# raadyn/aztotmd

Hardware: AMD Instinct MI355X
Metric: ns_per_day (higher is better)
Workload: dtype f64; 1 GPU; 1 000 188 Ar, LJ rc 8.5 A, FCC 63^3 a=5.735 jitter 0.15, dt 1 fs, NVE, init_vel zero (BASELINE config '1 000 000 Ar LJ', SURVEY C4); n_atoms=1000188, n_cells=68921, decomposition=single GPU, transport=single GPU, rccl_ranks=0, pair_variant=0, sort_interval=105, sort_violations=0, pair_lists=1, cells_without_list=0, kernel_timing=off

## Files before the change

aztotmd_amd/api.py:

```python
import ctypes as C
import enum
import os
import subprocess

import numpy as np

_HERE = os.path.dirname(os.path.abspath(__file__))
_LIB = None

STAT_FIELDS = ("step", "time", "engTot", "engKin", "engVdW", "engCoul", "engElecField", "engTemp", "engPot", "temperature",
               "posMom", "negMom", "posCross", "negCross", "pressure", "pairs_dropped", "n_cells", "nose_chit", "nose_conint",
               "engBond", "engAngle", "engCoulRec", "engCoulConst", "sort_interval", "sort_violations", "pair_lists", "cells_without_list", "rebuilds", "skin")


class AztotError(RuntimeError):
    def __init__(self, code, msg):
        super().__init__("aztot error %d: %s" % (code, msg))
        self.code = code


class _Species(C.Structure):
    _fields_ = [("name", C.c_char * 8), ("mass_amu", C.c_double), ("charge", C.c_double), ("frozen", C.c_int32),
                ("radA", C.c_double), ("radB", C.c_double), ("mxEng", C.c_double)]

# ... 92 lines not shown
           "aztot_adf_setup", "aztot_adf_sample", "aztot_adf_reset", "aztot_adf_shape", "aztot_adf_edges", "aztot_adf_counts", "aztot_adf_values",
           "aztot_adf_neighbours",
           "aztot_sk_setup", "aztot_sk_sample", "aztot_sk_reset", "aztot_sk_shape", "aztot_sk_vectors", "aztot_sk_amplitudes", "aztot_sk_sums", "aztot_sk_values",
           "aztot_boo_setup", "aztot_boo_sample", "aztot_boo_reset", "aztot_boo_shape", "aztot_boo_per_atom", "aztot_boo_qlm", "aztot_boo_counts", "aztot_boo_values",
           "aztot_last_error", "aztot_version")

RDF_KINDS = {"species": 0, "nuclei": 1}
CN_KINDS = {"species": 0, "nuclei": 1}


class DebugBit(enum.IntFlag):
    DBG_BUILD_PHASE_MASK = 3
    DBG_ALWAYS_CLEANUP = 4
    DBG_FOLD_DRIFT = 8
    DBG_NO_FOLD_DRIFT = 16
    DBG_KICK_EVERY_STEP = 128
    DBG_LARGE_KICK_PATH = 256
    DBG_GENERIC_PAIR = 512
    DBG_KEEP_VDW_CUT_TEST = 1024
    DBG_STAGE_ONLY = 2048
    DBG_SLAB_GRAPH = 4096
    DBG_FIXED_INTERVAL = 8192
    DBG_OVERLAP_HALO = 16384
    DBG_NO_LISTS = 32768
    DBG_SHORT_LISTS = 65536
    DBG_NO_FUSE_NEXT = 131072
    DBG_FUSE_NEXT = 262144
    DBG_CHECK_EVERY_ATOM = 524288
    DBG_LIST_STATS = 2097152
    DBG_KICK_POST_SPLIT = 4194304
# ... 670 lines not shown
```

aztotmd_amd/csrc/device_md.h:

```cpp
#pragma once
#include <cstdint>

namespace aztot {

constexpr int kSpecCap = 16;

struct AtomArrays
{
    double *x, *y, *z;
    double *vx, *vy, *vz;
    double *fx, *fy, *fz;
    double *U, *rad;
    int32_t *type;
    int32_t *id;
};

struct RefPos { double *x, *y, *z; };

struct SpecTable
{
    double mass[kSpecCap], charge[kSpecCap], rMhdt[kSpecCap];
    double radA[kSpecCap], radB[kSpecCap], mxEng[kSpecCap];
    int32_t charged[kSpecCap], frozen[kSpecCap];
};
// ... 48 lines not shown

struct SplitArgs
{
    int n = 1;
    double *fx = nullptr, *fy = nullptr, *fz = nullptr;
    int32_t* arrived = nullptr;
    int capacity = 0;
};

enum DebugBit : unsigned
{
    DBG_BUILD_PHASE_MASK = 3,
    DBG_ALWAYS_CLEANUP = 4,
    DBG_FOLD_DRIFT = 8,
    DBG_NO_FOLD_DRIFT = 16,
    DBG_KICK_EVERY_STEP = 128,
    DBG_LARGE_KICK_PATH = 256,
    DBG_GENERIC_PAIR = 512,
    DBG_KEEP_VDW_CUT_TEST = 1024,
    DBG_STAGE_ONLY = 2048,
    DBG_SLAB_GRAPH = 4096,
    DBG_FIXED_INTERVAL = 8192,
    DBG_OVERLAP_HALO = 16384,
    DBG_NO_LISTS = 32768,
    DBG_SHORT_LISTS = 65536,
    DBG_NO_FUSE_NEXT = 131072,
    DBG_FUSE_NEXT = 262144,
    DBG_CHECK_EVERY_ATOM = 524288,
    DBG_LIST_STATS = 2097152,
    DBG_KICK_POST_SPLIT = 4194304,
// ... 107 lines not shown
```

aztotmd_amd/csrc/engine.h:

```cpp
#pragma once
#include <hip/hip_runtime.h>

#include <algorithm>
#include <memory>
#include <stdexcept>
#include <string>
#include <vector>

#include "device_md.h"
#include "device_resources.h"
#include "list_store.h"
#include "model.h"
#include "msg_layout.h"
#include "samplers.h"

namespace aztot {

struct Counts;
struct PairLists; struct PairLaunch;

struct ArgError : std::runtime_error
{
    using std::runtime_error::runtime_error;
};
// ... 151 lines not shown

    double lastMom_[6] = {0, 0, 0, 0, 0, 0};
    double pressure_ = 0.0;
    long long lastPresStep_ = 0;

    std::unique_ptr<Samplers> samplers_;

    struct BufState { int cur; double* xyz[2][3]; double* alt[2][3]; };
    struct LaunchNotes
    {
        int pairBlocksUsed = 0;
        int blocksEver = 0;
        bool ekinFromPair = false;
        bool lastStepEquil = false;
    } notes_;
    struct GraphSlot { BufState before, after; LaunchNotes notes; hipGraph_t graph = nullptr; hipGraphExec_t exec = nullptr; };
    void adopt_launch_notes(const LaunchNotes& n) { const int ever = std::max(notes_.blocksEver, n.blocksEver); notes_ = n; notes_.blocksEver = ever; }
    std::vector<GraphSlot> graphs_;
    int graphCycle_ = 0;
    bool capturing_ = false;
    void drop_graphs();
    BufState buf_state() const;
    GraphSlot* graph_for_state(int cycle);
    int graph_cycle() const;
    bool can_graph() const;
    void set_buf_state(const BufState& b);

    bool lazyKick_ = false;
    bool kickOwed_ = false;
    bool fuseEpilogue_ = false;
    bool fuseNow_ = false;
// ... 40 lines not shown
```

aztotmd_amd/csrc/engine.hip:

```cpp
#include "engine.h"

#include <algorithm>
#include <cmath>
#include <array>
#include <cstring>
#include <cstddef>
#include <cstdio>
#include <cstdlib>
#include <stdexcept>
#include <tuple>

#include "exchange.h"
#include "bonded.hip.h"
#include "ewald.hip.h"
#include "kernels.hip.h"
#include "pair_tile.hip.h"
#include "pair_list.hip.h"
#include "rdf.hip.h"
#include "cn.hip.h"
#include "adf.hip.h"
#include "sk.hip.h"
#include "tcf.hip.h"
#include "slab.hip.h"

// ... 480 lines not shown
    PairLists probe;
    probe.candCap = probe.candLds = probe.stageLds = candCapNew; probe.iterCap = probe.iterLds = iterCapNew; probe.recBytes = pair_list_rec_bytes(P); probe.waves = waves;
    while (candCapNew > kListMinCand && (pair_list_lds_bytes(P, probe) > ldsMax_ || build_lists_lds_bytes(probe) > ldsMax_))
    {
        candCapNew -= 64;
        probe.candCap = probe.candLds = probe.stageLds = candCapNew;
    }
    while (iterCapNew > 2 * kListMinIter && build_lists_lds_bytes(probe) > ldsMax_) { iterCapNew -= 8; probe.iterCap = probe.iterLds = iterCapNew; }
    const size_t nc = (size_t)P.nCellLocal;
    cand = mem_.alloc<uint32_t>(nc * candCapNew, true, stream_);
    meta = mem_.alloc<int32_t>(4 * nc, false, stream_);
    pairs = mem_.alloc<uint16_t>(nc * (size_t)waves * (size_t)iterCapNew * kWave, true, stream_);
    report = mem_.alloc<int32_t>(LR_COUNT, true, stream_); rel = mem_.alloc<float4>((size_t)capacity_ + kWave, true, stream_);
    candCap = candCapNew; iterCap = iterCapNew;
    candLds = stageLds = candCapNew; iterLds = iterCapNew;
    {
        std::vector<int32_t> mx(4 * nc, 0);
        const int ncy = P.nc[1], ncz = P.nc[2];
        for (size_t c = 0; c < nc; c++)
        {
            const int cz = (int)(c % ncz), cy = (int)((c / ncz) % ncy), lx = (int)(c / ((size_t)ncy * ncz));
            mx[4 * c] = -1; mx[4 * c + 1] = lx | (cy << 10) | (cz << 20);
        }
        HIP_CHECK(hipMemcpyAsync(meta, mx.data(), sizeof(int32_t) * 4 * nc, hipMemcpyHostToDevice, stream_));
        HIP_CHECK(hipStreamSynchronize(stream_));
    }
    on = true;
    if (std::getenv("AZTOT_VERBOSE"))
        std::fprintf(stderr, "aztot: pair lists for %zu cells: %d candidates, %d iterations per cell (%.1f MB), LDS %zu B (list kernel) / %zu B (builder)\n", nc, candCap, iterCap,
                     (double)(nc * ((size_t)candCap * 4 + (size_t)iterCap * 128)) / 1e6, pair_list_lds_bytes(P, pair_lists()), build_lists_lds_bytes(pair_lists()));
// ... 12 lines not shown

void ListStore::release() noexcept
{
    if (stream_) (void)hipStreamSynchronize(stream_);
    mem_.release();
    cand = nullptr; meta = nullptr; pairs = nullptr; report = nullptr; rel = nullptr;
    on = false;
}

PairLists ListStore::pair_lists() const
{
    PairLists pl;
    if (on)
    {
        pl.cand = cand; pl.meta = meta; pl.pairs = pairs; pl.noList = report;
        pl.candCap = candCap; pl.iterCap = iterCap; pl.candLds = candLds; pl.stageLds = stageLds; pl.iterLds = iterLds; pl.recBytes = pair_list_rec_bytes(*P_); pl.entryScale = pair_list_entry_scale(*P_); pl.waves = waves;
        pl.rel = rel;
    }
    return pl;
}

int ListStore::tile_records_for(int maxT) const
{
    constexpr size_t kLdsBlock = 1280;
    PairLists L = pair_lists();
    const bool roomy = P_->nranks == 1 && capacity_ <= 2 * kFuseKickMaxAtoms;
    const int need = std::max(4 * kWave, std::min(candCap, roomy ? maxT + maxT / 16 + 4 : maxT + maxT / 100 + 1));
    if (need <= 4 * kWave) return need;
    L.candLds = need;
    const size_t blocks = (pair_list_lds_bytes(*P_, L) + kLdsBlock - 1) / kLdsBlock;
    int best = need;
    for (int c = need + 1; c <= candCap; c++)
    {
        L.candLds = c;
        if ((pair_list_lds_bytes(*P_, L) + kLdsBlock - 1) / kLdsBlock > blocks) break;
        best = c;
    }
    return best;
}

int ListStore::stage_records_for(int maxStaged) const
{
    return std::max(4 * kWave, std::min(candCap, (maxStaged + maxStaged / 16 + 4 + 127) & ~127));
}

void ListStore::lds_for(const int32_t* rep, int& candLdsNew, int& stageLdsNew, int& iterLdsNew) const
{
    candLdsNew = tile_records_for(rep[LR_MAX_TILE]);
    stageLdsNew = stage_records_for(rep[LR_MAX_STAGED]);
    iterLdsNew = std::max(2 * kListMinIter, std::min(iterCap, (rep[LR_MAX_ITERS] + rep[LR_MAX_ITERS] / 8 + 2 + 7) & ~7));
}

bool ListStore::tighten(const int32_t* rep)
{
    if (rep[LR_TILE_FULL] != 0 || rep[LR_LIST_FULL] != 0 || rep[LR_KEPT_FULL] != 0 || rep[LR_MAX_STAGED] <= 0) return false;
    int c, s, i;
    lds_for(rep, c, s, i);
    if (c >= candLds && s >= stageLds && i >= iterLds) return false;
    candLds = std::min(candLds, c); stageLds = std::min(stageLds, s); iterLds = std::min(iterLds, i);
    return true;
}

ListStore::Verdict ListStore::adapt(const int32_t* rep, unsigned debug)
{
    Verdict v;
    const bool frozen = debug & DBG_SHORT_LISTS;
    if (debug & DBG_LIST_STATS)
    {
        std::fprintf(stderr, "aztot: per cell: %.2f list iterations, %.1f candidates staged, %.1f kept, %.2f atoms\n", (double)rep[LR_SUM_ITERS] / rep[LR_RECORDED],
                     (double)rep[LR_SUM_STAGED] / rep[LR_RECORDED], (double)rep[LR_SUM_CANDS] / rep[LR_RECORDED], (double)rep[LR_SUM_ATOMS] / rep[LR_RECORDED]);
        HIP_CHECK(hipMemset(&report[LR_SUM_ITERS], 0, sizeof(int32_t) * 4));
    }
    HIP_CHECK(hipMemsetAsync(&report[LR_UNLISTED], 0, sizeof(int32_t) * 2, stream_));
    HIP_CHECK(hipMemsetAsync(&report[LR_TILE_FULL], 0, sizeof(int32_t) * 3, stream_));
    const int tileFull = rep[LR_TILE_FULL], keptFull = rep[LR_KEPT_FULL], listFull = rep[LR_LIST_FULL], recorded = rep[LR_RECORDED], unlisted = rep[LR_UNLISTED];
    if (std::getenv("AZTOT_VERBOSE"))
        std::fprintf(stderr, "aztot: lists recorded since the last look: %d cells, %d of them without a list (%d: staging full, %d: tile full, %d: list full); most staged %d of %d (LDS %d), largest tile %d (LDS %d), longest list %d of %d (LDS %d)\n",
                     recorded, unlisted, tileFull, keptFull, listFull, rep[LR_MAX_STAGED], candCap, stageLds, rep[LR_MAX_TILE], candLds, rep[LR_MAX_ITERS], iterCap, iterLds);
    int candLdsNew, stageLdsNew, iterLdsNew;
    lds_for(rep, candLdsNew, stageLdsNew, iterLdsNew);
    if (tileFull > 0) stageLdsNew = std::min(candCap, std::max(stageLdsNew, stageLds + 128));
    if (keptFull > 0) candLdsNew = std::min(candCap, std::max(candLdsNew, candLds + 32));
    if (listFull > 0) iterLdsNew = std::min(iterCap, std::max(iterLdsNew, iterLds + 8));
    if (frozen) { candLdsNew = candLds; stageLdsNew = stageLds; iterLdsNew = iterLds; }
    const int wWant = std::max(waves, waves_wanted((double)rep[LR_MAX_TILE], rep[LR_MAX_ITERS]));
    if (wWant > waves && !forcedWaves_ && !frozen)
    {
        const int itersNew = std::max(2 * kListMinIter, ((int)(rep[LR_MAX_ITERS] * (double)waves / wWant * 1.3) + 8 + 7) & ~7);
        const int candNew = std::max(candCap, kListMinCand * wWant);
        waves = wWant;
        regrow(candNew, itersNew);
        v.rebuild = v.launchChanged = true;
        return v;
    }
    const bool capFull = (tileFull > 0 && stageLds == candCap) || (keptFull > 0 && candLds == candCap) || (listFull > 0 && iterLds == iterCap);
    if (capFull && !frozen && (double)(tileFull + keptFull + listFull) > ((P_->nranks == 1 && growths < 3) ? 0.0 : 0.0005 * (double)recorded))
    {
        const int candNew = tileFull + keptFull > 0 ? std::min(kListCandMax, (candCap * 3 / 2 + 63) & ~63) : candCap;
        const int itersNew = listFull > 0 ? std::min(kListIterMax, (iterCap * 2 + 7) & ~7) : iterCap;
        v.launchChanged = true;
// ... 203 lines not shown
    return variant;
}

PairLaunch Engine::pair_launch(const StepParams& Q) { return PairLaunch{Q, S_, dPots_, cur(), dCounts_, dCellStart_, dPartials_, maxBlocks_, stream_}; }

void Engine::launch_pair()
{
    const int variant = pair_variant();
    int splitBlocks = 0;
    if (variant == 2)
    {
        StepParams Q = P_;
        Q.fuseKick = fuseNow_ ? KICK_SECOND : KICK_NONE;
        const PairLaunch C = pair_launch(Q);
        const bool wantEnergies = stepsLeftInRun_ == 0 || (debug_ & DBG_ENERGIES_EVERY_STEP);
        const PairLists pl = lists_.pair_lists();
        if (overlapHalo_)
        {
            const int plane = P_.nc[1] * P_.nc[2], hw = P_.hw[0];
            PairRange in, lo, hi;
            in.first = 2 * hw * plane; in.n = (P_.ncxLocal - 4 * hw) * plane;
            lo.first = hw * plane; lo.n = hw * plane;
            hi.first = (P_.ncxLocal - 2 * hw) * plane; hi.n = hw * plane;
            const bool lists = candMode_ == 2 && pl.cand;
            int nb = 0;
            auto run = [&](PairRange& r) {
                r.blockBase = nb;
                if (lists)
                {
                    nb += launch_pair_list(C, r, pl, NextStep(), wantEnergies);
// ... 37 lines not shown
                if (fuseNext_) { nx.xn = altXyz_[cur_][0]; nx.yn = altXyz_[cur_][1]; nx.zn = altXyz_[cur_][2]; }
                if (fuseNext_ && fuseNextTstat_) { nx.photons = dPhotons_; nx.uvx = dUvx_; nx.uvy = dUvy_; nx.uvz = dUvz_; pairClosedStep_ = true; }
                else nx.pendingAfter = lazyKick_ ? 1 : -1;
                const bool fold = foldKick_ && skipCleanup && !fuseNext_ && !wantEnergies;
                foldKick_ = false;
                StepParams QL = Q;
                const bool foldDrift = fold && foldDriftOk_;
                if (fold) { QL.fuseKick = foldDrift ? KICK_DRIFT : KICK_BOTH; nx.pendingAfter = 0; kickFolded_ = !foldDrift; }
                if (foldDrift)
                {
                    nx.xd = altXyz_[cur_][0]; nx.yd = altXyz_[cur_][1]; nx.zd = altXyz_[cur_][2];
                    nx.driftBlocks = div_up(div_up(capacity_, 2), kBlock);
                    if (profile_ && !capturing_) timers_.count("fold_drift");
                }
                const PairLaunch CL = pair_launch(QL);
                timed("pair_list", [&] { splitBlocks = launch_pair_list(CL, PairRange(), pl, nx, wantEnergies); });
                if (!skipCleanup)
                    timed("pair_cleanup", [&] { splitBlocks += launch_pair_cleanup(C, PairRange(), pl, nx); });
                if (fuseNext_ || foldDrift)
                {
                    AtomArrays& A = cur();
                    std::swap(A.x, altXyz_[cur_][0]); std::swap(A.y, altXyz_[cur_][1]); std::swap(A.z, altXyz_[cur_][2]);
                    preIntegrated_ = true;
                }
            }
            else
                timed("pair_tile", [&] { launch_pair_tile(C, PairRange(), pl, 0, NextStep(), split_); });
        }
    }
    else
// ... 443 lines not shown
    const bool slabGraph = nranks_ > 1 && ownedXch_ && (debug_ & DBG_SLAB_GRAPH) && !(P_.nEq > 0 || P_.tstat == AZTOT_TSTAT_NOSE);
    const bool worthIt = capacity_ <= 2 * kFuseKickMaxAtoms || (debug_ & DBG_GRAPH_ALWAYS);
    return opt_.use_graph && worthIt && (nranks_ == 1 || slabGraph) && !profile_ && !equil_phase();
}

Engine::GraphSlot* Engine::graph_for_state(int cycle)
{
    if (graphCycle_ != cycle) { drop_graphs(); graphCycle_ = cycle; }
    const BufState now = buf_state();
    for (GraphSlot& g : graphs_)
        if (g.before.cur == now.cur && g.before.xyz[0][0] == now.xyz[0][0] && g.before.xyz[1][0] == now.xyz[1][0]) return &g;
    GraphSlot g;
    g.before = now;
    const int sinceBefore = sinceSort_;
    const LaunchNotes notesBefore = notes_;
    HIP_CHECK(hipStreamBeginCapture(stream_, hipStreamCaptureModeThreadLocal));
    capturing_ = true;
    try
    {
        sinceSort_ = kNoSort;
        preIntegrated_ = false;
        kickFolded_ = false;
        for (int k = 0; k < cycle; k++) { stepsLeftInRun_ = cycle - 1 - k; launch_step_kernels(); }
    }
    catch (...)
    {
        hipGraph_t broken = nullptr;
        (void)hipStreamEndCapture(stream_, &broken);
        if (broken) (void)hipGraphDestroy(broken);
        capturing_ = false;
        preIntegrated_ = false;
        kickFolded_ = false;
        sinceSort_ = sinceBefore;
        set_buf_state(now);
        adopt_launch_notes(notesBefore);
        throw;
    }
    capturing_ = false;
    HIP_CHECK(hipStreamEndCapture(stream_, &g.graph));
    HIP_CHECK(hipGraphInstantiate(&g.exec, g.graph, nullptr, nullptr, 0));
    g.after = buf_state();
    g.notes = notes_;
    set_buf_state(now);
    adopt_launch_notes(notesBefore);
    sinceSort_ = sinceBefore;
    stepsLeftInRun_ = 0;
    graphs_.push_back(g);
    return &graphs_.back();
}

void Engine::run_steps(int nsteps)
{
    int done = 0;
    const bool carryOn = lazyOn_ && (nranks_ == 1 || carryAgreed_) && lists_.on && listsValid_ && lazyK_ > 1 && sinceSort_ < kNoSort / 2 && pair_variant() == 2;
    if (!carryOn) sinceSort_ = kNoSort;
    preIntegrated_ = false;
    while (carryOn && done < nsteps && sinceSort_ < lazyK_ - 1) { stepsLeftInRun_ = nsteps - 1 - done; launch_step_kernels(); done++; }
    const int cycle = graph_cycle();
    if (can_graph() && nsteps - done >= cycle)
    {
        sinceSort_ = kNoSort;
        while (nsteps - done >= cycle)
        {
            GraphSlot* slot = graph_for_state(cycle);
            HIP_CHECK(hipGraphLaunch(slot->exec, stream_));
            done += cycle;
            hostStep_ += cycle;
            rebuilds_ += (lazyOn_ && lazyK_ > 1) ? 1 : cycle;
            set_buf_state(slot->after);
            adopt_launch_notes(slot->notes);
            sinceSort_ = kNoSort;
        }
    }
    preIntegrated_ = false;
    for (; done < nsteps; done++) { stepsLeftInRun_ = nsteps - 1 - done; launch_step_kernels(); }
    stepsLeftInRun_ = 0;
}

void Engine::prepare_next_call()
{
    if (!lazyOn_ || !lazyMeasured_) return;
    if (lists_.on && lazyK_ > 1 && !listsValid_ && sinceSort_ == 0 && pair_variant() == 2)
    {
        P_.cycleStep = 0;
        HIP_CHECK(hipMemsetAsync(&lists_.report[LR_UNLISTED_NOW], 0, sizeof(int32_t), stream_));
        launch_build_lists(pair_launch(P_), PairRange(), lists_.pair_lists());
        check_launch("list building");
        sync();
        int32_t rep[LR_COUNT];
        HIP_CHECK(hipMemcpy(rep, lists_.report, sizeof(rep), hipMemcpyDeviceToHost));
        unlistedState_ = (rep[LR_UNLISTED_NOW] == 0) ? 1 : 2;
        if (!(debug_ & DBG_SHORT_LISTS) && lists_.tighten(rep)) drop_graphs();
        if (nranks_ > 1)
        {
            int32_t h[HI_COUNT];
            post_count_exchange();
            HIP_CHECK(hipStreamSynchronize(stream_));
            HIP_CHECK(hipMemcpy(h, dHaloInfo_, sizeof(h), hipMemcpyDeviceToHost));
            haloInfoPending_ = false;
            adopt_halo_info(h);
        }
        listsValid_ = true;
    }
    if (nranks_ > 1)
    {
        double cannot = (lists_.on && listsValid_ && lazyK_ > 1 && pair_variant() == 2) ? 0.0 : 1.0;
        xch_->allreduce_sum(&cannot, 1, stream_);
// ... 286 lines not shown
```

aztotmd_amd/csrc/list_store.h:

```cpp
#pragma once
#include "device_resources.h"
#include "model.h"

namespace aztot {

struct StepParams; struct PairLists;

struct ListStore
{
    struct Verdict
    {
        bool rebuild = false;
        bool launchChanged = false;
    };

    bool on = false;
    uint32_t* cand = nullptr;
    int32_t* meta = nullptr;
    uint16_t* pairs = nullptr;
    int32_t* report = nullptr;
    float4* rel = nullptr;
    int candCap = 0, iterCap = 0;
    int candLds = 0, iterLds = 0;
    int stageLds = 0;
    int waves = 1;
    int growths = 0;

    void create(const StepParams& P, const Model& m, const aztot_options& opt, int capacity, double listRadius, hipStream_t stream, int rank);
    void regrow(int candCap, int iterCap);
    void release() noexcept;
    PairLists pair_lists() const;
    void lds_for(const int32_t* rep, int& candLds, int& stageLds, int& iterLds) const;
    bool tighten(const int32_t* rep);
    Verdict adapt(const int32_t* rep, unsigned debug);

private:
    void allocate(int candCap, int iterCap);
    int tile_records_for(int maxT) const;
    int stage_records_for(int maxStaged) const;
    int waves_wanted(double tileRecords, int iters) const;
    DeviceArena mem_;
    const StepParams* P_ = nullptr;
    hipStream_t stream_ = nullptr;
    int capacity_ = 0, rank_ = 0;
    int forcedWaves_ = 0;
    size_t ldsMax_ = 0;
};

}
```

aztotmd_amd/csrc/pair_list.hip.h:

```cpp
#pragma once
#include <type_traits>
#include "pair_tile.hip.h"

namespace aztot {

constexpr int kListPreload = 5;
constexpr int kListMinCand = 64 * kListPreload;
__host__ __device__ inline int list_preload(int candLds) { return candLds <= 4 * kWave ? 4 : kListPreload; }
constexpr int kListMinIter = 16;
constexpr int kListMaxSlices = 32;

constexpr int kListMaxWaves = 4;
__host__ __device__ inline int list_atoms_per_wave(int nAtoms, int W) { return (nAtoms + W - 1) >> (W >> 1); }
__host__ __device__ inline int list_slices(int nAtomsOfWave) { const int n = kWave / (nAtomsOfWave > 0 ? nAtomsOfWave : 1); return n > kListMaxSlices ? kListMaxSlices : (n < 1 ? 1 : n); }

inline bool pair_list_tab_mode(const StepParams& P) { return P.potSet == POTSET_ONE_FAMILY && !P.single_lj; }
inline size_t pair_list_lds_bytes(const StepParams& P, const PairLists& L)
{
    const bool tab = pair_list_tab_mode(P);
    const bool generic = !P.single_lj && P.potSet == POTSET_GENERIC;
    const bool radii = !P.single_lj && !tab;
    size_t b = (size_t)(L.candLds + 1) * 24;
    if (tab) b += sizeof(double) * kLjSpecMax * kLjSpecMax * kPairTabStride + (((size_t)L.candLds + 1 + 15) & ~(size_t)15);
    if (radii) b += sizeof(double) * (size_t)(L.candLds + 1);
// ... 58 lines not shown
    {
        if (N.cnt->lazyViolated == 0) N.cnt->lazyViolated = P.cycleStep + 1;
        N.cnt->lazyViolatedEver = 1;
    }
    if (__any(cross != 0))
    {
#pragma unroll
        for (int d = 0; d < 6; d++) if (cross & (1 << d)) atomicAdd(&N.st->specCross[t * 6 + d], 1ULL);
        const double m = S.mass[t];
        next_wall_sum(m * (-vx), cross & 1, 1, 0, partials, maxBlocks, pb); next_wall_sum(m * vx, cross & 2, 2, 1, partials, maxBlocks, pb);
        next_wall_sum(m * (-vy), cross & 4, 4, 2, partials, maxBlocks, pb); next_wall_sum(m * vy, cross & 8, 8, 3, partials, maxBlocks, pb);
        next_wall_sum(m * (-vz), cross & 16, 16, 4, partials, maxBlocks, pb); next_wall_sum(m * vz, cross & 32, 32, 5, partials, maxBlocks, pb);
    }
}

template <int MODE, int VDW, bool ENG, bool MULTI, bool TSTAT = false, int PRE = kListPreload>
__global__ __launch_bounds__(MULTI ? kWave * kListMaxWaves : kWave) void k_pair_list(StepParams P, SpecTable S, const DevPot* __restrict__ pots, AtomArrays A,
                                                     const int32_t* __restrict__ cellStart, int firstCell, int nCellsRun,
                                                     double* __restrict__ partials, int maxBlocks, const Counts* __restrict__ counts, int blockBase, PairLists L,
                                                     NextStep N)
{
    constexpr bool kOneSpecies = pair_mode_one_species(MODE);
    constexpr bool kRadii = pair_mode_reads_radii(MODE);
    constexpr bool kTab = pair_mode_has_table(MODE);
    constexpr int RECB = 24;
    constexpr int ESCALE = (MODE == PM_ONE_LJ) ? 1 : 24;
    constexpr int kTabDoubles = kTab ? kLjSpecMax * kLjSpecMax * kPairTabStride : 0;
    extern __shared__ double ldsList[];
    double* const pairTab = ldsList;
    uint8_t* const ttypT = (uint8_t*)(ldsList + kTabDoubles);
    char* const tb = (char*)(ldsList + kTabDoubles) + (kTab ? ((L.candLds + 1 + 15) & ~15) : 0);
    double* const trad = (double*)(tb + (size_t)(L.candLds + 1) * RECB);
    uint8_t* const ttyp0 = (uint8_t*)(trad + (L.candLds + 1));

    const int lane = threadIdx.x & (kWave - 1), wave = MULTI ? (int)(threadIdx.x >> 6) : 0;
    const int W = MULTI ? L.waves : 1;
    const int per = (nCellsRun + 7) >> 3;
    const int cr = (blockIdx.x & 7) * per + (blockIdx.x >> 3);
    double eV = 0.0, eC = 0.0, dropped = 0.0, eK = 0.0;
    NextAcc nacc;
    if (N.xn) next_acc_clear(nacc);
    const int cell = firstCell + min(cr, nCellsRun - 1);
    const uint32_t* const myList = L.cand + (size_t)cell * L.candCap + lane;
    const uint4* const pl = (const uint4*)(L.pairs + ((size_t)cell * W + wave) * L.iterCap * kWave) + lane;
    uint32_t ent[PRE];
#pragma unroll
    for (int u = 0; u < PRE; u++) ent[u] = myList[(wave + u * W) * kWave];
    uint4 w = pl[0];
    uint4 w1 = pl[kWave];
    const int4 mx = ((const int4*)L.meta)[cell];
    unsigned long long runBits = 0ULL, maxBits = 0ULL;
    if (P.fuseKick == KICK_DRIFT) { runBits = N.cnt->cycMaxRun; maxBits = N.cnt->maxStep2; }
    asm volatile("" ::: "memory");
    const bool violated = P.nranks == 1 && !P.optimistic && slack_violated(P, counts);
    int meta = mx.x;
    if (violated || cr >= nCellsRun || !list_usable(L, meta)) meta = -1;
    if (meta > 0)
    {
        const int T = meta & 0xFFF, nIter = (meta >> 12) & 0xFF;
        const int ncy = P.nc[1], ncz = P.nc[2];
        const int lx = mx.y & 1023, cy = (mx.y >> 10) & 1023, cz = (mx.y >> 20) & 1023;
        const int ib = mx.z;
        const double cc0 = (lx + P.cx0) * P.csz[0] + 0.5 * P.csz[0], cc1 = cy * P.csz[1] + 0.5 * P.csz[1], cc2 = cz * P.csz[2] + 0.5 * P.csz[2];
        const DevPot lj = pots[0];
        if (kTab)
        {
            const int np = P.nSpec * P.nSpec;
            if (threadIdx.x < np)
            {
                const DevPot v = pots[lane];
                const int a = lane / P.nSpec, b = lane - a * P.nSpec;
                double* q = pairTab + lane * kPairTabStride;
                q[0] = v.p0; q[1] = v.p1; q[2] = v.p2; q[3] = v.p3; q[4] = v.p4;
                q[5] = v.type ? v.r2cut : -1.0;
// ... 81 lines not shown
        if (threadIdx.x == 0)
        {
            char* const r = tb;
            *(double*)r = -1e30; *(double*)(r + 8) = -1e30; *(double*)(r + 16) = -1e30;
            if (kTab) ttypT[0] = 0;
            if (kRadii) trad[0] = 1.0;
            if (MODE == PM_GENERIC) ttyp0[0] = 0;
        }
        __syncthreads();

        PairAcc acc = {0, 0, 0, 0, 0, 0};
        int nDropHalf = 0;
        double ljDropR2 = P.ljDropR2;
        if (kTab) asm volatile("" : "+v"(ljDropR2));
        const PairHot hot = kTab ? pair_hot_in_vgprs(P, lj) : (MODE == PM_ONE_LJ ? pair_hot_lj_in_vgprs(P, lj) : pair_hot(P, lj));
        const int nChunks = (nIter + 7) >> 3;
        double xj, yj, zj, radj = 0.0;
        int tj = 0;
        auto fetch = [&](uint32_t en, double& x, double& y, double& z, int& ty, double& rd) {
            const uint32_t ko = en * ESCALE;
            x = *(const double*)(tb + ko);
            y = *(const double*)(tb + ko + 8);
            z = *(const double*)(tb + ko + 16);
            if (kTab) ty = ttypT[en];
            if (kRadii) rd = trad[en];
            if (MODE == PM_GENERIC) ty = ttyp0[en];
        };
        fetch(nIter > 0 ? (w.x & 0xFFFFu) : dummyOff, xj, yj, zj, tj, radj);
        for (int c = 0; c < nChunks; c++)
        {
            uint4 wn = w1;
            if (c + 2 < nChunks) w1 = pl[(c + 2) * kWave];
            const uint32_t ww[5] = {w.x, w.y, w.z, w.w, wn.x};
#pragma unroll
            for (int u = 0; u < 8; u++)
            {
                const int t = c * 8 + u;
                if (t >= nIter) break;
                uint32_t kn = ((u + 1) & 1) ? (ww[(u + 1) >> 1] >> 16) : (ww[(u + 1) >> 1] & 0xFFFFu);
                if (u == 7 && c + 1 >= nChunks) kn = dummyOff;
                double xn, yn, zn, radn = 0.0;
                int tn = 0;
                fetch(kn, xn, yn, zn, tn, radn);
                {
                    const double dx = xi - xj, dy = yi - yj, dz = zi - zj;
                    const double r2 = dx * dx + dy * dy + dz * dz;
                    pair_body<MODE, VDW, true>(P, S, pots, lj, pairTab, true, dx, dy, dz, r2, ti, tj, radi, radj, ljDropR2, nDropHalf, acc, hot);
                }
                xj = xn; yj = yn; zj = zn; tj = tn; radj = radn;
            }
            w = wn;
        }
        if (MODE != PM_GENERIC) acc.dropped += 0.5 * (double)nDropHalf;

        if (NS == 4)
// ... 369 lines not shown
                myList[n] = entry;
            }
            kept += __popcll(mask);
        };
        if (entInRegs)
        {
#pragma unroll
            for (int u = 0; u < kBuildEntRegs; u++) if (u * kWave < T) keep_chunk(u * kWave, te[u]);
        }
        else
            for (int q0 = 0; q0 < T; q0 += kWave) keep_chunk(q0, tent[min(q0 + lane, T - 1)]);
        const int Tpad = max((kept + kWave - 1) & ~(kWave - 1), list_preload(L.candLds) * W * kWave);
        for (int q = kept + lane; q < Tpad; q += kWave) myList[q] = (uint32_t)ib | (0x15u << 26);
        __builtin_amdgcn_wave_barrier();
    }
    const bool keptFull = usable && kept > L.candLds;
    if (keptFull) usable = false;
    if (usable)
    {
        const int slot = (lane * rcpNS) >> 16, slice = lane - slot * NS;
        for (int w = 0; w < W; w++)
        {
            const int atom = w * aw + slot;
            int off = 0, cnt = 0;
            if (slot < aw && atom < nthis) { off = entN[atom]; cnt = entC[atom]; }
            const uint16_t* const src = hits + off;
            uint4* const out = (uint4*)(L.pairs + ((size_t)cell * W + w) * L.iterCap * kWave) + lane;
            for (int c = 0; c * 8 < nIter; c++)
            {
                uint32_t v[8];
#pragma unroll
                for (int u = 0; u < 8; u++)
                {
                    const int e = (c * 8 + u) * NS + slice;
                    v[u] = (e < cnt) ? (uint32_t)remap[src[e]] : 0u;
                }
                out[c * kWave] = make_uint4(v[0] | (v[1] << 16), v[2] | (v[3] << 16), v[4] | (v[5] << 16), v[6] | (v[7] << 16));
            }
        }
    }
    if (lane == 0)
    {
        L.meta[4 * cell] = usable ? (kept | (nIter << 12) | (NS << 20)) : -1;
        L.meta[4 * cell + 2] = ib;
        L.meta[4 * cell + 3] = nthis | (rcpNS << 12);
        if (T > L.noList[LR_MAX_STAGED]) atomicMax(&L.noList[LR_MAX_STAGED], T);
        if (kept > L.noList[LR_MAX_TILE]) atomicMax(&L.noList[LR_MAX_TILE], kept);
        if (usable && nIter > L.noList[LR_MAX_ITERS]) atomicMax(&L.noList[LR_MAX_ITERS], nIter);
        if (P.debugMask & DBG_LIST_STATS)
        {
            atomicAdd(&L.noList[LR_SUM_ITERS], nIter); atomicAdd(&L.noList[LR_SUM_CANDS], kept); atomicAdd(&L.noList[LR_SUM_ATOMS], nthis); atomicAdd(&L.noList[LR_SUM_STAGED], T);
        }
        if (!usable) { atomicAdd(&L.noList[LR_UNLISTED], 1); atomicAdd(&L.noList[LR_UNLISTED_NOW], 1); atomicAdd(&L.noList[keptFull ? LR_KEPT_FULL : LR_LIST_FULL], 1); }
    }
}

inline void launch_build_lists(const PairLaunch& C, PairRange R, PairLists L)
{
    pair_range_default(C.P, R);
    if (R.n == 0) return;
    const BuildLds G(L.stageLds, L.iterLds, L.waves);
    hipLaunchKernelGGL(k_build_lists, dim3(pair_range_grid(R.n)), dim3(kWave), G.bytes(), C.stream, C.P, C.cellStart, R.first, R.n, L);
}
inline size_t build_lists_lds_bytes(const PairLists& L) { return BuildLds(L.stageLds, L.iterLds, L.waves).bytes(); }

template <int MODE, int VDW>
inline void launch_pair_list_as(const PairLaunch& C, PairRange R, PairLists L, NextStep N, bool energies)
{
    const size_t lds = pair_list_lds_bytes(C.P, L);
    const dim3 grid(pair_range_grid(R.n)), block(kWave * L.waves);
    constexpr bool kCanFuseTstat = !pair_mode_reads_radii(MODE);
    const bool four = list_preload(L.candLds) == 4;
#define AZTOT_LAUNCH_LIST_PRE(E, M, T, G) hipLaunchKernelGGL((k_pair_list<MODE, VDW, E, M, T, G>), grid, block, lds, C.stream, C.P, C.S, C.pots, C.A, C.cellStart, R.first, R.n, C.partials, C.maxBlocks, C.cnt, R.blockBase, L, N)
#define AZTOT_LAUNCH_LIST(E, M, T) do { if (four) AZTOT_LAUNCH_LIST_PRE(E, M, T, 4); else AZTOT_LAUNCH_LIST_PRE(E, M, T, kListPreload); } while (0)
    if (N.photons)
    {
        if (energies || !kCanFuseTstat) throw std::runtime_error("k_pair_list: the thermostat cannot be fused into this launch");
        if (L.waves == 1) AZTOT_LAUNCH_LIST(false, false, kCanFuseTstat); else AZTOT_LAUNCH_LIST(false, true, kCanFuseTstat);
    }
    else if (L.waves == 1) { if (energies) AZTOT_LAUNCH_LIST(true, false, false); else AZTOT_LAUNCH_LIST(false, false, false); }
    else { if (energies) AZTOT_LAUNCH_LIST(true, true, false); else AZTOT_LAUNCH_LIST(false, true, false); }
#undef AZTOT_LAUNCH_LIST
#undef AZTOT_LAUNCH_LIST_PRE
}

inline int launch_pair_list(const PairLaunch& C, PairRange R, PairLists L, NextStep N = NextStep(), bool energies = true)
{
    pair_range_default(C.P, R);
    if (R.n == 0) return 0;
// ... 15 lines not shown
```

aztotmd_amd/csrc/pair_tile.hip.h:

```cpp
#pragma once
#include "kernels.hip.h"

namespace aztot {

constexpr int kTileCap = 320;
constexpr int kTilePad = 16;
constexpr int kTileLds = kTileCap + kTilePad;
static_assert(kTileLds % 32 == 16, "coordinate arrays must be staggered by half the LDS banks");

typedef float float4_t __attribute__((ext_vector_type(4)));

enum PairMode { PM_GENERIC = 0, PM_ONE_LJ = 1, PM_TAB = 2, PM_TAB_EWALD = 3, PM_ONE_SURK = 4, PM_TAB_FENNELL = 5 };
enum PairVdw { VDW_ANY = 0, VDW_LNJS = 1, VDW_BUCK = 2, VDW_P746 = 3, VDW_BMHS = 4, VDW_MIXED = 5, VDW_LJ_NOCUT = 6, VDW_SURK = 7 };
constexpr bool pair_mode_has_table(int mode) { return mode == PM_TAB || mode == PM_TAB_EWALD || mode == PM_TAB_FENNELL; }
constexpr bool pair_mode_reads_radii(int mode) { return mode == PM_GENERIC || mode == PM_ONE_SURK; }
constexpr bool pair_mode_one_species(int mode) { return mode == PM_ONE_LJ || mode == PM_ONE_SURK; }
constexpr bool pair_mode_ewald(int mode) { return mode == PM_TAB_EWALD; }
constexpr bool pair_mode_fennell(int mode) { return mode == PM_TAB_FENNELL; }
constexpr bool pair_vdw_is_lj(int vdw) { return vdw == VDW_LNJS || vdw == VDW_LJ_NOCUT; }
constexpr bool pair_vdw_no_cut_test(int vdw) { return vdw == VDW_LJ_NOCUT; }
constexpr bool pair_vdw_mixed(int vdw) { return vdw == VDW_MIXED; }


inline bool pair_tile_supported(const StepParams& P)
// ... 290 lines not shown
    if (MODE != PM_GENERIC) acc.dropped += 0.5 * (double)nDropHalf;
}

enum ListReport : int
{
    LR_UNLISTED = 0,
    LR_RECORDED = 1,
    LR_UNLISTED_NOW = 2,
    LR_MAX_TILE = 3,
    LR_MAX_ITERS = 4,
    LR_TILE_FULL = 5,
    LR_LIST_FULL = 6,
    LR_KEPT_FULL = 7,
    LR_SUM_ITERS = 8, LR_SUM_CANDS = 9, LR_SUM_ATOMS = 10, LR_SUM_STAGED = 11,
    LR_MAX_STAGED = 12,
    LR_COUNT = 16,
    LR_NONE = -1
};
struct PairLists
{
    uint32_t* cand = nullptr;
    int32_t* meta = nullptr;
    uint16_t* pairs = nullptr;
    int32_t* noList = nullptr;
    int32_t candCap = 0;
    int32_t iterCap = 0;
    int32_t candLds = 0;
    int32_t stageLds = 0;
    int32_t iterLds = 0;
    int32_t waves = 1;
    int32_t recBytes = 0;
    int32_t entryScale = 0;
    const float4* rel = nullptr;
};
__device__ __forceinline__ bool list_usable(const PairLists& L, int header) { return header >= 0 && (header & 0xFFF) <= L.candLds; }

__device__ __forceinline__ int wave_max_int(int v)
{
#pragma unroll
    for (int o = kWave >> 1; o >= 1; o >>= 1) v = max(v, __shfl_xor(v, o, kWave));
    return v;
}

struct NextStep
{
    double *xn = nullptr, *yn = nullptr, *zn = nullptr;
    RefPos R0{};
// ... 470 lines not shown
```

Measured before the change: 843.2 ns/day.

## Pack pair-list neighbour entries into one byte when tiles hold at most 255 records

Adds a narrow one-byte pair-list entry format, used when a cell's candidate tile has at most 255 records, there is one wave per cell and the run is single-rank. Each 16-byte list vector then holds 16 neighbours instead of 8, which halves list memory traffic and the number of list loads in the force kernel. The list store switches between formats adaptively: it re-records the lists when the format changes, falls back to wide entries permanently on overflow, and keeps the chosen format in each captured graph slot. The cost is extra host-side state and rebuild logic, plus a candidate LDS size forced to the minimum in the narrow case.

```diff
diff --git a/aztotmd_amd/api.py b/aztotmd_amd/api.py
--- a/aztotmd_amd/api.py
+++ b/aztotmd_amd/api.py
@@ -130,6 +130,7 @@
     DBG_ALWAYS_CLEANUP = 4
     DBG_FOLD_DRIFT = 8
     DBG_NO_FOLD_DRIFT = 16
+    DBG_WIDE_ENTRIES = 32
     DBG_KICK_EVERY_STEP = 128
     DBG_LARGE_KICK_PATH = 256
     DBG_GENERIC_PAIR = 512
diff --git a/aztotmd_amd/csrc/device_md.h b/aztotmd_amd/csrc/device_md.h
--- a/aztotmd_amd/csrc/device_md.h
+++ b/aztotmd_amd/csrc/device_md.h
@@ -86,6 +86,7 @@
     DBG_ALWAYS_CLEANUP = 4,
     DBG_FOLD_DRIFT = 8,
     DBG_NO_FOLD_DRIFT = 16,
+    DBG_WIDE_ENTRIES = 32,
     DBG_KICK_EVERY_STEP = 128,
     DBG_LARGE_KICK_PATH = 256,
     DBG_GENERIC_PAIR = 512,
diff --git a/aztotmd_amd/csrc/engine.h b/aztotmd_amd/csrc/engine.h
--- a/aztotmd_amd/csrc/engine.h
+++ b/aztotmd_amd/csrc/engine.h
@@ -189,7 +189,7 @@
         bool ekinFromPair = false;
         bool lastStepEquil = false;
     } notes_;
-    struct GraphSlot { BufState before, after; LaunchNotes notes; hipGraph_t graph = nullptr; hipGraphExec_t exec = nullptr; };
+    struct GraphSlot { BufState before, after; LaunchNotes notes; hipGraph_t graph = nullptr; hipGraphExec_t exec = nullptr; int entryBytes = 2; };
     void adopt_launch_notes(const LaunchNotes& n) { const int ever = std::max(notes_.blocksEver, n.blocksEver); notes_ = n; notes_.blocksEver = ever; }
     std::vector<GraphSlot> graphs_;
     int graphCycle_ = 0;
diff --git a/aztotmd_amd/csrc/engine.hip b/aztotmd_amd/csrc/engine.hip
--- a/aztotmd_amd/csrc/engine.hip
+++ b/aztotmd_amd/csrc/engine.hip
@@ -518,6 +518,7 @@
     report = mem_.alloc<int32_t>(LR_COUNT, true, stream_); rel = mem_.alloc<float4>((size_t)capacity_ + kWave, true, stream_);
     candCap = candCapNew; iterCap = iterCapNew;
     candLds = stageLds = candCapNew; iterLds = iterCapNew;
+    entryBytes = entryNext = 2;
     {
         std::vector<int32_t> mx(4 * nc, 0);
         const int ncy = P.nc[1], ncz = P.nc[2];
@@ -560,7 +561,8 @@
     if (on)
     {
         pl.cand = cand; pl.meta = meta; pl.pairs = pairs; pl.noList = report;
-        pl.candCap = candCap; pl.iterCap = iterCap; pl.candLds = candLds; pl.stageLds = stageLds; pl.iterLds = iterLds; pl.recBytes = pair_list_rec_bytes(*P_); pl.entryScale = pair_list_entry_scale(*P_); pl.waves = waves;
+        pl.candCap = candCap; pl.iterCap = iterCap; pl.candLds = candLds; pl.stageLds = stageLds; pl.iterLds = iterLds; pl.recBytes = pair_list_rec_bytes(*P_); pl.waves = waves;
+        pl.entryBytes = entryBytes; pl.entryScale = entryBytes == 1 ? 1 : pair_list_entry_scale(*P_);
         pl.rel = rel;
     }
     return pl;
@@ -571,7 +573,8 @@
     constexpr size_t kLdsBlock = 1280;
     PairLists L = pair_lists();
     const bool roomy = P_->nranks == 1 && capacity_ <= 2 * kFuseKickMaxAtoms;
-    const int need = std::max(4 * kWave, std::min(candCap, roomy ? maxT + maxT / 16 + 4 : maxT + maxT / 100 + 1));
+    int need = std::max(4 * kWave, std::min(candCap, roomy ? maxT + maxT / 16 + 4 : maxT + maxT / 100 + 1));
+    if (maxT <= 255 && P_->nranks == 1 && waves == 1) need = 4 * kWave;
     if (need <= 4 * kWave) return need;
     L.candLds = need;
     const size_t blocks = (pair_list_lds_bytes(*P_, L) + kLdsBlock - 1) / kLdsBlock;
@@ -595,14 +598,29 @@
     candLdsNew = tile_records_for(rep[LR_MAX_TILE]);
     stageLdsNew = stage_records_for(rep[LR_MAX_STAGED]);
     iterLdsNew = std::max(2 * kListMinIter, std::min(iterCap, (rep[LR_MAX_ITERS] + rep[LR_MAX_ITERS] / 8 + 2 + 7) & ~7));
-}
-
-bool ListStore::tighten(const int32_t* rep)
-{
+    if (entryNext == 1 && ((iterLdsNew + 15) & ~15) <= iterCap) iterLdsNew = (iterLdsNew + 15) & ~15;
+}
+
+bool ListStore::narrow_fits(int maxTile, int candLdsNew, int wavesNew) const
+{
+    return P_->nranks == 1 && !(P_->debugMask & DBG_WIDE_ENTRIES) && !wideForGood_ && wavesNew == 1 && list_preload(candLdsNew) == 4 && maxTile <= 255;
+}
+
+bool ListStore::tighten(const int32_t* rep, bool* formatChanged)
+{
+    if (formatChanged) *formatChanged = false;
     if (rep[LR_TILE_FULL] != 0 || rep[LR_LIST_FULL] != 0 || rep[LR_KEPT_FULL] != 0 || rep[LR_MAX_STAGED] <= 0) return false;
     int c, s, i;
     lds_for(rep, c, s, i);
-    if (c >= candLds && s >= stageLds && i >= iterLds) return false;
+    bool changed = false;
+    if (entryNext == 2 && narrow_fits(rep[LR_MAX_TILE], std::min(candLds, c), waves))
+    {
+        entryNext = 1;
+        lds_for(rep, c, s, i);
+        changed = true;
+        if (formatChanged) *formatChanged = true;
+    }
+    if (c >= candLds && s >= stageLds && i >= iterLds) return changed;
     candLds = std::min(candLds, c); stageLds = std::min(stageLds, s); iterLds = std::min(iterLds, i);
     return true;
 }
@@ -613,9 +631,11 @@
     const bool frozen = debug & DBG_SHORT_LISTS;
     if (debug & DBG_LIST_STATS)
     {
-        std::fprintf(stderr, "aztot: per cell: %.2f list iterations, %.1f candidates staged, %.1f kept, %.2f atoms\n", (double)rep[LR_SUM_ITERS] / rep[LR_RECORDED],
-                     (double)rep[LR_SUM_STAGED] / rep[LR_RECORDED], (double)rep[LR_SUM_CANDS] / rep[LR_RECORDED], (double)rep[LR_SUM_ATOMS] / rep[LR_RECORDED]);
+        std::fprintf(stderr, "aztot: per cell: %.2f list iterations, %.1f candidates staged, %.1f kept, %.2f atoms; %.1f %% of the cells walk more than 16 iterations (%d-byte entries)\n",
+                     (double)rep[LR_SUM_ITERS] / rep[LR_RECORDED], (double)rep[LR_SUM_STAGED] / rep[LR_RECORDED], (double)rep[LR_SUM_CANDS] / rep[LR_RECORDED],
+                     (double)rep[LR_SUM_ATOMS] / rep[LR_RECORDED], 100.0 * (double)rep[LR_OVER_16] / rep[LR_RECORDED], entryBytes);
         HIP_CHECK(hipMemset(&report[LR_SUM_ITERS], 0, sizeof(int32_t) * 4));
+        HIP_CHECK(hipMemset(&report[LR_OVER_16], 0, sizeof(int32_t)));
     }
     HIP_CHECK(hipMemsetAsync(&report[LR_UNLISTED], 0, sizeof(int32_t) * 2, stream_));
     HIP_CHECK(hipMemsetAsync(&report[LR_TILE_FULL], 0, sizeof(int32_t) * 3, stream_));
@@ -630,6 +650,18 @@
     if (listFull > 0) iterLdsNew = std::min(iterCap, std::max(iterLdsNew, iterLds + 8));
     if (frozen) { candLdsNew = candLds; stageLdsNew = stageLds; iterLdsNew = iterLds; }
     const int wWant = std::max(waves, waves_wanted((double)rep[LR_MAX_TILE], rep[LR_MAX_ITERS]));
+    const int wavesNew = (wWant > waves && !forcedWaves_ && !frozen) ? wWant : waves;
+    if (entryNext == 1 && (rep[LR_MAX_TILE] > 255 || keptFull > 0 || !narrow_fits(rep[LR_MAX_TILE], candLdsNew, wavesNew)))
+    {
+        entryNext = 2; wideForGood_ = true;
+        v.rebuild = v.launchChanged = true;
+    }
+    else if (entryNext == 2 && !frozen && tileFull + keptFull + listFull == 0 && narrow_fits(rep[LR_MAX_TILE], candLdsNew, wavesNew))
+    {
+        entryNext = 1;
+        v.launchChanged = true;
+        lds_for(rep, candLdsNew, stageLdsNew, iterLdsNew);
+    }
     if (wWant > waves && !forcedWaves_ && !frozen)
     {
         const int itersNew = std::max(2 * kListMinIter, ((int)(rep[LR_MAX_ITERS] * (double)waves / wWant * 1.3) + 8 + 7) & ~7);
@@ -863,6 +895,7 @@
         Q.fuseKick = fuseNow_ ? KICK_SECOND : KICK_NONE;
         const PairLaunch C = pair_launch(Q);
         const bool wantEnergies = stepsLeftInRun_ == 0 || (debug_ & DBG_ENERGIES_EVERY_STEP);
+        if (candMode_ == 1 && lists_.on && !overlapHalo_) lists_.begin_recording();
         const PairLists pl = lists_.pair_lists();
         if (overlapHalo_)
         {
@@ -930,6 +963,7 @@
                     if (profile_ && !capturing_) timers_.count("fold_drift");
                 }
                 const PairLaunch CL = pair_launch(QL);
+                if (profile_ && !capturing_ && pl.entryBytes == 1) timers_.count("narrow_lists");
                 timed("pair_list", [&] { splitBlocks = launch_pair_list(CL, PairRange(), pl, nx, wantEnergies); });
                 if (!skipCleanup)
                     timed("pair_cleanup", [&] { splitBlocks += launch_pair_cleanup(C, PairRange(), pl, nx); });
@@ -1403,6 +1437,7 @@
     g.before = now;
     const int sinceBefore = sinceSort_;
     const LaunchNotes notesBefore = notes_;
+    const int entryBytesBefore = lists_.entryBytes;
     HIP_CHECK(hipStreamBeginCapture(stream_, hipStreamCaptureModeThreadLocal));
     capturing_ = true;
     try
@@ -1421,6 +1456,7 @@
         preIntegrated_ = false;
         kickFolded_ = false;
         sinceSort_ = sinceBefore;
+        lists_.entryBytes = entryBytesBefore;
         set_buf_state(now);
         adopt_launch_notes(notesBefore);
         throw;
@@ -1430,6 +1466,8 @@
     HIP_CHECK(hipGraphInstantiate(&g.exec, g.graph, nullptr, nullptr, 0));
     g.after = buf_state();
     g.notes = notes_;
+    g.entryBytes = lists_.entryBytes;
+    lists_.entryBytes = entryBytesBefore;
     set_buf_state(now);
     adopt_launch_notes(notesBefore);
     sinceSort_ = sinceBefore;
@@ -1458,6 +1496,7 @@
             rebuilds_ += (lazyOn_ && lazyK_ > 1) ? 1 : cycle;
             set_buf_state(slot->after);
             adopt_launch_notes(slot->notes);
+            lists_.entryBytes = slot->entryBytes;
             sinceSort_ = kNoSort;
         }
     }
@@ -1472,14 +1511,20 @@
     if (lists_.on && lazyK_ > 1 && !listsValid_ && sinceSort_ == 0 && pair_variant() == 2)
     {
         P_.cycleStep = 0;
-        HIP_CHECK(hipMemsetAsync(&lists_.report[LR_UNLISTED_NOW], 0, sizeof(int32_t), stream_));
-        launch_build_lists(pair_launch(P_), PairRange(), lists_.pair_lists());
-        check_launch("list building");
-        sync();
         int32_t rep[LR_COUNT];
-        HIP_CHECK(hipMemcpy(rep, lists_.report, sizeof(rep), hipMemcpyDeviceToHost));
-        unlistedState_ = (rep[LR_UNLISTED_NOW] == 0) ? 1 : 2;
-        if (!(debug_ & DBG_SHORT_LISTS) && lists_.tighten(rep)) drop_graphs();
+        auto record = [&] {
+            HIP_CHECK(hipMemsetAsync(&lists_.report[LR_UNLISTED_NOW], 0, sizeof(int32_t), stream_));
+            lists_.begin_recording();
+            launch_build_lists(pair_launch(P_), PairRange(), lists_.pair_lists());
+            check_launch("list building");
+            sync();
+            HIP_CHECK(hipMemcpy(rep, lists_.report, sizeof(rep), hipMemcpyDeviceToHost));
+            unlistedState_ = (rep[LR_UNLISTED_NOW] == 0) ? 1 : 2;
+        };
+        record();
+        bool formatChanged = false;
+        if (!(debug_ & DBG_SHORT_LISTS) && lists_.tighten(rep, &formatChanged)) drop_graphs();
+        if (formatChanged) record();
         if (nranks_ > 1)
         {
             int32_t h[HI_COUNT];
diff --git a/aztotmd_amd/csrc/list_store.h b/aztotmd_amd/csrc/list_store.h
--- a/aztotmd_amd/csrc/list_store.h
+++ b/aztotmd_amd/csrc/list_store.h
@@ -25,13 +25,16 @@
     int stageLds = 0;
     int waves = 1;
     int growths = 0;
+    int entryBytes = 2, entryNext = 2;
 
     void create(const StepParams& P, const Model& m, const aztot_options& opt, int capacity, double listRadius, hipStream_t stream, int rank);
     void regrow(int candCap, int iterCap);
     void release() noexcept;
     PairLists pair_lists() const;
     void lds_for(const int32_t* rep, int& candLds, int& stageLds, int& iterLds) const;
-    bool tighten(const int32_t* rep);
+    bool tighten(const int32_t* rep, bool* formatChanged = nullptr);
+    bool narrow_fits(int maxTile, int candLdsNew, int wavesNew) const;
+    void begin_recording() { entryBytes = entryNext; }
     Verdict adapt(const int32_t* rep, unsigned debug);
 
 private:
@@ -44,6 +47,7 @@
     hipStream_t stream_ = nullptr;
     int capacity_ = 0, rank_ = 0;
     int forcedWaves_ = 0;
+    bool wideForGood_ = false;
     size_t ldsMax_ = 0;
 };
 
diff --git a/aztotmd_amd/csrc/pair_list.hip.h b/aztotmd_amd/csrc/pair_list.hip.h
--- a/aztotmd_amd/csrc/pair_list.hip.h
+++ b/aztotmd_amd/csrc/pair_list.hip.h
@@ -96,7 +96,7 @@
     }
 }
 
-template <int MODE, int VDW, bool ENG, bool MULTI, bool TSTAT = false, int PRE = kListPreload>
+template <int MODE, int VDW, bool ENG, bool MULTI, bool TSTAT = false, int PRE = kListPreload, int EB = 2>
 __global__ __launch_bounds__(MULTI ? kWave * kListMaxWaves : kWave) void k_pair_list(StepParams P, SpecTable S, const DevPot* __restrict__ pots, AtomArrays A,
                                                      const int32_t* __restrict__ cellStart, int firstCell, int nCellsRun,
                                                      double* __restrict__ partials, int maxBlocks, const Counts* __restrict__ counts, int blockBase, PairLists L,
@@ -106,7 +106,9 @@
     constexpr bool kRadii = pair_mode_reads_radii(MODE);
     constexpr bool kTab = pair_mode_has_table(MODE);
     constexpr int RECB = 24;
-    constexpr int ESCALE = (MODE == PM_ONE_LJ) ? 1 : 24;
+    static_assert(EB == 2 || (EB == 1 && !MULTI && PRE == 4), "one-byte list entries: one wave per cell and the four-group tile only");
+    constexpr int ESCALE = (MODE == PM_ONE_LJ && EB == 2) ? 1 : 24;
+    constexpr int VPC = 16 / EB;
     constexpr int kTabDoubles = kTab ? kLjSpecMax * kLjSpecMax * kPairTabStride : 0;
     extern __shared__ double ldsList[];
     double* const pairTab = ldsList;
@@ -129,7 +131,8 @@
 #pragma unroll
     for (int u = 0; u < PRE; u++) ent[u] = myList[(wave + u * W) * kWave];
     uint4 w = pl[0];
-    uint4 w1 = pl[kWave];
+    uint4 w1 = make_uint4(0u, 0u, 0u, 0u);
+    if (EB == 2) w1 = pl[kWave];
     const int4 mx = ((const int4*)L.meta)[cell];
     unsigned long long runBits = 0ULL, maxBits = 0ULL;
     if (P.fuseKick == KICK_DRIFT) { runBits = N.cnt->cycMaxRun; maxBits = N.cnt->maxStep2; }
@@ -140,6 +143,11 @@
     if (meta > 0)
     {
         const int T = meta & 0xFFF, nIter = (meta >> 12) & 0xFF;
+        if (EB == 1)
+        {
+            if (nIter > VPC) w1 = pl[kWave];
+            asm volatile("" ::: "memory");
+        }
         const int ncy = P.nc[1], ncz = P.nc[2];
         const int lx = mx.y & 1023, cy = (mx.y >> 10) & 1023, cz = (mx.y >> 20) & 1023;
         const int ib = mx.z;
@@ -251,7 +259,7 @@
         double ljDropR2 = P.ljDropR2;
         if (kTab) asm volatile("" : "+v"(ljDropR2));
         const PairHot hot = kTab ? pair_hot_in_vgprs(P, lj) : (MODE == PM_ONE_LJ ? pair_hot_lj_in_vgprs(P, lj) : pair_hot(P, lj));
-        const int nChunks = (nIter + 7) >> 3;
+        const int nChunks = (nIter + VPC - 1) / VPC;
         double xj, yj, zj, radj = 0.0;
         int tj = 0;
         auto fetch = [&](uint32_t en, double& x, double& y, double& z, int& ty, double& rd) {
@@ -263,19 +271,21 @@
             if (kRadii) rd = trad[en];
             if (MODE == PM_GENERIC) ty = ttyp0[en];
         };
-        fetch(nIter > 0 ? (w.x & 0xFFFFu) : dummyOff, xj, yj, zj, tj, radj);
+        fetch(nIter > 0 ? (w.x & (EB == 1 ? 0xFFu : 0xFFFFu)) : dummyOff, xj, yj, zj, tj, radj);
         for (int c = 0; c < nChunks; c++)
         {
             uint4 wn = w1;
             if (c + 2 < nChunks) w1 = pl[(c + 2) * kWave];
             const uint32_t ww[5] = {w.x, w.y, w.z, w.w, wn.x};
 #pragma unroll
-            for (int u = 0; u < 8; u++)
-            {
-                const int t = c * 8 + u;
+            for (int u = 0; u < VPC; u++)
+            {
+                const int t = c * VPC + u;
                 if (t >= nIter) break;
-                uint32_t kn = ((u + 1) & 1) ? (ww[(u + 1) >> 1] >> 16) : (ww[(u + 1) >> 1] & 0xFFFFu);
-                if (u == 7 && c + 1 >= nChunks) kn = dummyOff;
+                uint32_t kn;
+                if (EB == 1) kn = (ww[(u + 1) >> 2] >> (8 * ((u + 1) & 3))) & 0xFFu;
+                else kn = ((u + 1) & 1) ? (ww[(u + 1) >> 1] >> 16) : (ww[(u + 1) >> 1] & 0xFFFFu);
+                if (u == VPC - 1 && c + 1 >= nChunks) kn = dummyOff;
                 double xn, yn, zn, radn = 0.0;
                 int tn = 0;
                 fetch(kn, xn, yn, zn, tn, radn);
@@ -675,7 +685,8 @@
         for (int q = kept + lane; q < Tpad; q += kWave) myList[q] = (uint32_t)ib | (0x15u << 26);
         __builtin_amdgcn_wave_barrier();
     }
-    const bool keptFull = usable && kept > L.candLds;
+    const bool narrow = L.entryBytes == 1;
+    const bool keptFull = usable && (kept > L.candLds || (narrow && kept > 255));
     if (keptFull) usable = false;
     if (usable)
     {
@@ -687,6 +698,22 @@
             if (slot < aw && atom < nthis) { off = entN[atom]; cnt = entC[atom]; }
             const uint16_t* const src = hits + off;
             uint4* const out = (uint4*)(L.pairs + ((size_t)cell * W + w) * L.iterCap * kWave) + lane;
+            if (narrow)
+            {
+                for (int c = 0; c * 16 < nIter; c++)
+                {
+                    uint32_t v[4] = {0u, 0u, 0u, 0u};
+#pragma unroll
+                    for (int u = 0; u < 16; u++)
+                    {
+                        const int e = (c * 16 + u) * NS + slice;
+                        const uint32_t r = (e < cnt) ? (uint32_t)remap[src[e]] : 0u;
+                        v[u >> 2] |= r << (8 * (u & 3));
+                    }
+                    out[c * kWave] = make_uint4(v[0], v[1], v[2], v[3]);
+                }
+                continue;
+            }
             for (int c = 0; c * 8 < nIter; c++)
             {
                 uint32_t v[8];
@@ -711,6 +738,7 @@
         if (P.debugMask & DBG_LIST_STATS)
         {
             atomicAdd(&L.noList[LR_SUM_ITERS], nIter); atomicAdd(&L.noList[LR_SUM_CANDS], kept); atomicAdd(&L.noList[LR_SUM_ATOMS], nthis); atomicAdd(&L.noList[LR_SUM_STAGED], T);
+            if (nIter > 16) atomicAdd(&L.noList[LR_OVER_16], 1);
         }
         if (!usable) { atomicAdd(&L.noList[LR_UNLISTED], 1); atomicAdd(&L.noList[LR_UNLISTED_NOW], 1); atomicAdd(&L.noList[keptFull ? LR_KEPT_FULL : LR_LIST_FULL], 1); }
     }
@@ -732,8 +760,10 @@
     const dim3 grid(pair_range_grid(R.n)), block(kWave * L.waves);
     constexpr bool kCanFuseTstat = !pair_mode_reads_radii(MODE);
     const bool four = list_preload(L.candLds) == 4;
-#define AZTOT_LAUNCH_LIST_PRE(E, M, T, G) hipLaunchKernelGGL((k_pair_list<MODE, VDW, E, M, T, G>), grid, block, lds, C.stream, C.P, C.S, C.pots, C.A, C.cellStart, R.first, R.n, C.partials, C.maxBlocks, C.cnt, R.blockBase, L, N)
-#define AZTOT_LAUNCH_LIST(E, M, T) do { if (four) AZTOT_LAUNCH_LIST_PRE(E, M, T, 4); else AZTOT_LAUNCH_LIST_PRE(E, M, T, kListPreload); } while (0)
+    const bool narrow = L.entryBytes == 1;
+    if (narrow && (!four || L.waves != 1)) throw std::runtime_error("k_pair_list: one-byte list entries need one wave per cell and a tile of at most 256 records");
+#define AZTOT_LAUNCH_LIST_PRE(E, M, T, G, B) hipLaunchKernelGGL((k_pair_list<MODE, VDW, E, M, T, G, B>), grid, block, lds, C.stream, C.P, C.S, C.pots, C.A, C.cellStart, R.first, R.n, C.partials, C.maxBlocks, C.cnt, R.blockBase, L, N)
+#define AZTOT_LAUNCH_LIST(E, M, T) do { if (narrow) AZTOT_LAUNCH_LIST_PRE(E, false, T, 4, 1); else if (four) AZTOT_LAUNCH_LIST_PRE(E, M, T, 4, 2); else AZTOT_LAUNCH_LIST_PRE(E, M, T, kListPreload, 2); } while (0)
     if (N.photons)
     {
         if (energies || !kCanFuseTstat) throw std::runtime_error("k_pair_list: the thermostat cannot be fused into this launch");
diff --git a/aztotmd_amd/csrc/pair_tile.hip.h b/aztotmd_amd/csrc/pair_tile.hip.h
--- a/aztotmd_amd/csrc/pair_tile.hip.h
+++ b/aztotmd_amd/csrc/pair_tile.hip.h
@@ -328,6 +328,7 @@
     LR_KEPT_FULL = 7,
     LR_SUM_ITERS = 8, LR_SUM_CANDS = 9, LR_SUM_ATOMS = 10, LR_SUM_STAGED = 11,
     LR_MAX_STAGED = 12,
+    LR_OVER_16 = 13,
     LR_COUNT = 16,
     LR_NONE = -1
 };
@@ -345,6 +346,7 @@
     int32_t waves = 1;
     int32_t recBytes = 0;
     int32_t entryScale = 0;
+    int32_t entryBytes = 2;
     const float4* rel = nullptr;
 };
 __device__ __forceinline__ bool list_usable(const PairLists& L, int header) { return header >= 0 && (header & 0xFFF) <= L.candLds; }
```

Result: faster. 913.0 ns/day (median of 6 runs) (+8.3%).
